# NVlabs/gbrl

Hardware: AMD Instinct MI355X
Metric: trees-fit/sec + predict rows/sec at batch=2^20, feat=128, depth=6, out=8 (higher is better)
Workload: dtype int32 fixed-point sums / f32 scores

## Files before the change

gbrl_amd/csrc/engine.h:

```cpp
#pragma once

#include <hip/hip_runtime.h>

#include <cstdint>
#include <stdexcept>
#include <array>
#include <initializer_list>
#include <chrono>
#include <cstring>
#include <string>
#include <unordered_map>
#include <vector>

#include "kernels.h"
#include "model.h"

namespace gbrl {

struct HipError : std::runtime_error { using std::runtime_error::runtime_error; };
struct NoDeviceError : std::runtime_error { using std::runtime_error::runtime_error; };
struct InvalidArgument : std::runtime_error { using std::runtime_error::runtime_error; };
struct Unsupported : std::runtime_error { using std::runtime_error::runtime_error; };

void hip_check(hipError_t e, const char *what);
// ... 233 lines not shown
    kern::PredictModel mirror_view();
    void finish(const char *launch, const char *phase, std::initializer_list<ReadBack> results);
    void run_predict(const PredictBatch &b, int start_tree, int stop_tree, float *out, bool out_dev);
    void run_continue(const PredictBatch &b, int start_tree, int stop_tree, const float *base, bool base_dev, float *out, bool out_dev);
    uint64_t cat_dict_token();
    void grow_tree(const detail::GrowCtx &c, std::vector<detail::HNode> &nodes, std::vector<int> &frontier, std::vector<int64_t> &acc,
                   double &leaf_scale);
    enum class SmallGrowth { Grown, NearTie, Unavailable };
    detail::StepTables upload_step_tables(const detail::GrowCtx &c, const detail::GrowDims &dims);
    SmallGrowth grow_small(const detail::GrowCtx &c, const detail::GrowDims &dims, const detail::StepTables &t, int blocks, detail::TreeBuilder &tb,
                           std::vector<int64_t> &acc, double &leaf_scale, const char *&why);
    void grow_levels(const detail::GrowCtx &c, const detail::GrowDims &dims, const detail::StepTables &t, detail::TreeBuilder &tb,
                     std::vector<int64_t> &acc, double &leaf_scale);
    detail::LevelWork level_workspace(const detail::GrowCtx &c, const detail::GrowDims &dims);
    void grow_levels_planned(const detail::GrowCtx &c, const detail::GrowDims &dims, const detail::StepTables &t, detail::LevelWork &w, detail::TreeBuilder &tb);
    void grow_levels_host(const detail::GrowCtx &c, const detail::GrowDims &dims, const detail::StepTables &t, detail::LevelWork &w, detail::TreeBuilder &tb,
                          detail::Stager &sta, detail::Stager &stb);
    detail::Level stage_level(const detail::GrowCtx &c, const detail::GrowDims &dims, detail::LevelWork &w, detail::TreeBuilder &tb, detail::Stager &sta, int depth,
                              std::vector<int> active);
    void level_histograms(const detail::GrowCtx &c, const detail::GrowDims &dims, const detail::LevelWork &w, const detail::Level &L);
    uint32_t score_select_level(const detail::GrowCtx &c, const detail::GrowDims &dims, const detail::StepTables &t, const detail::LevelWork &w, const detail::Level &L);
    void replay_near_ties(const detail::GrowCtx &c, const detail::GrowDims &dims, const detail::StepTables &t, const detail::LevelWork &w,
                          const std::vector<detail::HNode> &nodes, const detail::Level &L);
    void finish_leaves(const detail::GrowCtx &c, const detail::GrowDims &dims, const detail::LevelWork &w, detail::TreeBuilder &tb, detail::Stager &sta,
                       std::vector<int64_t> &acc, double &leaf_scale);
    uint32_t next_seq() { const uint32_t seq = ++level_seq_; return seq ? seq : ++level_seq_; }
    bool device_categorical_candidates(const char *dcells, const char *hcells, int N, int Fc, int B,
                                       std::vector<detail::CatCandidate> &cat_cands, std::vector<int> &cat_classes, bool launch_only = false,
                                       const float *dgrads = nullptr, int D = 0);
    void sharded_categorical_ranking(const char *hcat, const float *hgrads, int N, int Fc, int D, int B, std::vector<detail::CatCandidate> &cat_cands,
                                     std::vector<uint16_t> &h_catcodes, std::vector<int> &cat_classes);
    void numeric_thresholds(const float *dobs, int N, int F, int B, long long n_global, const uint32_t *d_kt, float *d_thr,
                            uint32_t *d_thrkeys, DevBuf &root_le_buf, const uint32_t **root_le_out, int pass1_chunks = 0, uint16_t *d_codes_out = nullptr,
                            bool *codes_written = nullptr);
    void read_step_hooks();
    bool fused_prep_applies(int N, int F, long long n_global) const;
    void check_prepared_model(const char *what) const;
    void check_prepared_dataset(const char *what, const PreparedDataset *ds) const;
    void step_prepared_run(const PreparedDataset *ds, const float *dgrads, const int32_t *d_rows, int m, const int32_t *cols = nullptr, int n_cols = 0);
    void begin_step_profile();
    void sync_code_bins(const PreparedDataset &ds);
    void check_code_range(const PreparedDataset &ds, const char *what, int start_tree, int stop_tree);
    kern::CodeTables sync_code_tables(const PreparedDataset &ds);
    NumericPrep prepare_numeric(PrepBuffers &pb, const float *dobs, int N, int F, int Fc, long long n_global, bool prep_candidate, detail::FusedStats *fs);
    void run_grad_stats(detail::FusedStats &g, int N, long long &n_global);
    void grow_step_tree(const detail::StepData &d, std::vector<detail::HNode> &nodes, std::vector<int> &frontier, std::vector<int64_t> &acc, double &leaf_scale);
// ... 207 lines not shown
```

gbrl_amd/csrc/engine_candidates.hip:

```cpp
#include "engine_step_detail.h"

namespace gbrl {

namespace detail {

void spin_until_published(volatile uint32_t *flag, uint32_t seq, hipStream_t s, const char *what) {
    const double kSpinSeconds = [] { const char *e = hooks::raw(hooks::SPIN_SECONDS); const double v = e ? std::atof(e) : 0.0; return v > 0.0 ? v : 120.0; }();
    int idle = 0;
    std::chrono::steady_clock::time_point t0;
    bool timed = false;
    for (unsigned spins = 1; *flag != seq; ++spins) {
        if ((spins & 0x3fff) == 0) {
            const hipError_t q = hipStreamQuery(s);
            if (q == hipSuccess) { if (++idle > 64) throw HipError(std::string("internal: ") + what + " were not published"); }
            else if (q != hipErrorNotReady) hip_check(q, what);
            if (!timed) { t0 = std::chrono::steady_clock::now(); timed = true; }
            else if (std::chrono::duration<double>(std::chrono::steady_clock::now() - t0).count() > kSpinSeconds) {
                hip_check(hipStreamSynchronize(s), what);
                if (*flag == seq) break;
                throw HipError(std::string("timeout: ") + what + " did not arrive (stream drained, nothing published)");
            }
        }
    }
    std::atomic_thread_fence(std::memory_order_acquire);
// ... 584 lines not shown
                bisection_quantiles(cum);
            } else if (!has_coll_ && !force_sample_select_ && !force_radix_ && kern::sort_quantiles_fits(N, B)) {
                int64_t *d_cum = upload_cum(cum);
                const bool no_fuse = [] { const char *e = hooks::raw(hooks::SORT_NO_CODES); return e && e[0] == '1'; }();
                uint16_t *cdst = no_fuse ? nullptr : d_codes_out;
                kern::sort_quantiles(d_kt, N, F, d_cum, B, d_thrkeys, d_thr, s, cdst);
                if (cdst && codes_written) *codes_written = true;
                floats_done = true;
                last_quantile_fallback_ = false;
            } else if (!force_sample_select_ && B <= kern::radix_max_targets() && n_global < (1ll << 32)) {
                int64_t *d_cum = upload_cum(cum);
                void *d_rs = d_radix_state_.ensure(kern::radix_state_bytes(F, B));
                uint32_t *d_rp = static_cast<uint32_t *>(d_radix_partial_.ensure(kern::radix_partial_bytes(F)));
                uint32_t *d_rl = static_cast<uint32_t *>(d_qlists_.ensure(kern::radix_list_bytes(N, F)));
                kern::RadixComm comm{};
                if (has_coll_) {
                    comm.ctx = this;
                    comm.allreduce_sum_i64 = &Engine::radix_exchange_trampoline;
                    comm.stream_ordered = rccl_comm_ != nullptr;
                    comm.gbuf = static_cast<int64_t *>(d_counts_.ensure(sizeof(int64_t) * kern::radix_exchange_words(F)));
                    comm.partial_global = static_cast<uint32_t *>(d_radix_global_.ensure(kern::radix_global_partial_bytes(F)));
                }
                uint32_t *d_le = has_coll_ ? nullptr : static_cast<uint32_t *>(root_le_buf.ensure(sizeof(uint32_t) * (static_cast<size_t>(F) * B + F)));
                const int rc = kern::radix_select(d_kt, N, F, d_cum, B, d_rs, d_rp, d_rl, d_thrkeys, s, has_coll_ ? &comm : nullptr, pass1_chunks, d_le);
                if (root_le_out) *root_le_out = d_le;
                if (rc != 0) throw HipError(rc == 2 ? "allreduce failed" : "radix select failed");
                last_quantile_fallback_ = false;
            } else {
                fast_quantile = true;
                kern::QuantilePlan plan = kern::quantile_plan(N);
                if (has_coll_) { plan.sample = 4096; plan.n_split = kern::kQuantileMaxSplit; }
                const size_t all_keys = static_cast<size_t>(N) * F;
                const uint32_t max_elems = static_cast<uint32_t>(B > 256 ? all_keys : std::min<size_t>(all_keys, std::max<size_t>(1u << 20, all_keys / 4)));
                int64_t *d_cum = upload_cum(cum);
                uint32_t *d_split = static_cast<uint32_t *>(d_splitters_.ensure(sizeof(uint32_t) * 2 * static_cast<size_t>(F) * kern::kQuantileMaxSplit));
                uint32_t *d_split_bfs = d_split + static_cast<size_t>(F) * kern::kQuantileMaxSplit;
                uint32_t *d_cc = static_cast<uint32_t *>(d_ccounts_.ensure(sizeof(uint32_t) * static_cast<size_t>(plan.n_chunks) * F * kern::kQuantileClasses));
                uint32_t *d_coff = static_cast<uint32_t *>(d_c2l_.ensure(sizeof(uint32_t) * F * kern::kQuantileClasses));
                uint32_t *d_toff = static_cast<uint32_t *>(d_tgt_list_.ensure(sizeof(uint32_t) * 2 * static_cast<size_t>(F) * B));
                uint32_t *d_tlen = d_toff + static_cast<size_t>(F) * B;
                uint32_t *d_tr = static_cast<uint32_t *>(d_tgt_rank_.ensure(sizeof(uint32_t) * F * B));
                uint32_t *d_lists = static_cast<uint32_t *>(d_qlists_.ensure(sizeof(uint32_t) * max_elems));
                hip_check(hipMemsetAsync(d_coff, 0xff, sizeof(uint32_t) * F * kern::kQuantileClasses, s), "memset");
                hip_check(hipMemsetAsync(d_qflags, 0, sizeof(uint32_t) * 4, s), "memset");
                int64_t *d_gcounts = nullptr;
                if (has_coll_) {
                    const int S = 4096, SU = S * coll_.world_size;
// ... 65 lines not shown
```

gbrl_amd/csrc/engine_grow_detail.h:

```cpp
#pragma once
#include "engine_step_detail.h"

namespace gbrl {
namespace detail {

struct GrowDims {
    GrowDims(const GrowCtx &c, bool has_coll, int world_size, int rank, Engine::Parity parity);
    int max_front, max_nodes, max_chunks;
    bool l2_degenerate;
    size_t table_cap, stage_bytes;
    int hist_chunk_budget, hist_max_chunks;
    size_t n_acc, hist_node_elems, feat_elems;
    int coll_P, coll_Fs, coll_lo, own_slots;
    size_t ar_max_bytes;
    int am_parts;
    size_t am_cap;
    size_t res_bytes;
    bool near_on;
    float near_rel;
    int near_max_rows;
    bool reference_asked;
    bool event_results;
};

// ... 55 lines not shown
    std::vector<HCond> in_cond_;
};

struct LevelWork {
    int32_t *rows[2];
    int32_t *rows_scratch;
    bool iota_root = false;
    int cur = 0;
    bool ar_prefix = false;
    int32_t *partials;
    int64_t *hist_lvl[2];
    int64_t *hist_coll, *hist_recv, *gather;
    float *scores, *parent, *am_v, *am_s;
    int32_t *am_i, *am_n;
    int32_t *cursors;
    int64_t *leafacc;
    ResultBlock d_res;
    ResultBlock h_res;
    volatile uint32_t *h_flag;
    void *h_res_dev;
    uint32_t *d_flag;
    unsigned *d_pub_done;
    NodeSplit *resolved;
};

struct Level {
    int depth = 0, n_act = 0;
    std::vector<int> active, compute_ids;
    std::vector<int32_t> slot_map;
    ChunkTable hist;
    std::vector<Chunk> count_chunks, part_chunks;
    bool hist_direct = false, root_countless = false, ar_level = false, drop_derived = false;
    int root_mode = 1, lvl_slots = 0, lvl_lo = 0;
    int64_t *d_hist = nullptr;
    const int64_t *d_hist_prev = nullptr;
    Chunk *d_chunks, *d_count_chunks, *d_part_chunks;
    int32_t *d_chunk_begin, *d_slotmap, *d_sub_par, *d_sub_sib, *d_path_len, *d_path_slot, *d_path_bin, *d_isroot, *d_seg_starts, *d_n_locals;
    float *d_path_val;
};

}
}
```

gbrl_amd/csrc/engine_grow_levels.hip:

```cpp
#include "engine_grow_detail.h"

namespace gbrl {

using namespace detail;

void Engine::grow_levels(const GrowCtx &c, const GrowDims &dims, const StepTables &t, TreeBuilder &tb, std::vector<int64_t> &acc, double &leaf_scale) {
    hipStream_t s = stream_;
    const bool device_plan = c.oblivious && !has_coll_ && device_levels_requested() && c.MD > 0 && c.MD <= 11  &&
                             c.n_cand > 0 && !dims.l2_degenerate;
    Stager sta(pin_a_, d_stage_a_, dims.stage_bytes, s), stb(pin_b_, d_stage_b_, dims.stage_bytes, s);
    LevelWork w = level_workspace(c, dims);
    tb.reset(dims.max_nodes);
    kern::publish_pair(c.d_thr, c.pub_thr_dev, c.pub_thr_bytes, c.d_scales, c.pub_scales_dev, sizeof(kern::StepScales), s);
    if (device_plan) grow_levels_planned(c, dims, t, w, tb);
    else if (c.n_cand > 0 && !dims.l2_degenerate) grow_levels_host(c, dims, t, w, tb, sta, stb);
    finish_leaves(c, dims, w, tb, sta, acc, leaf_scale);
}

LevelWork Engine::level_workspace(const GrowCtx &c, const GrowDims &dims) {
    hipStream_t s = stream_;
    const int N = c.N, D = c.D, max_front = dims.max_front;
    LevelWork w{};
    w.rows[0] = static_cast<int32_t *>(d_rows_[0].ensure(sizeof(int32_t) * N));
    w.rows[1] = static_cast<int32_t *>(d_rows_[1].ensure(sizeof(int32_t) * N));
// ... 110 lines not shown
    hip_check(hipMemcpyAsync(h_res_all, d_res_all, res_bytes * MD, hipMemcpyDeviceToHost, s), "D2H tree results");
    hip_check(hipStreamSynchronize(s), "sync tree");
    hip_check(hipGetLastError(), "growth kernels");
    for (int depth = 0; depth < MD; ++depth) {
        const std::vector<int> active = tb.frontier;
        if (static_cast<int>(active.size()) != (1 << depth)) throw HipError("internal: level size mismatch");
        LevelOutcome lvl = tb.digest_level(active, level_block(h_res_all, depth), DigestMode{});
        if (lvl.stop || lvl.splitting.empty()) { if (!lvl.stop) tb.frontier.clear(); break; }
        w.cur ^= 1;
        tb.frontier = lvl.next;
    }
}

void Engine::grow_levels_host(const GrowCtx &c, const GrowDims &dims, const StepTables &t, LevelWork &w, TreeBuilder &tb, Stager &sta, Stager &stb) {
    hipStream_t s = stream_;
    const int N = c.N;
    for (int depth = 0; depth < c.MD; ++depth) {
        std::vector<int> active = tb.active_nodes();
        if (active.empty()) break;
        const Level L = stage_level(c, dims, w, tb, sta, depth, std::move(active));
        level_histograms(c, dims, w, L);
        const uint32_t seq = score_select_level(c, dims, t, w, L);
        if (dims.event_results) hip_check(hipEventRecord(ev_level_, s), "hipEventRecord");
        phase_begin();
        if (!L.part_chunks.empty())
            kern::partition_rows(w.rows[w.cur], w.rows[w.cur ^ 1], c.d_codes, c.d_kt, N, L.d_part_chunks, static_cast<int>(L.part_chunks.size()), w.resolved, w.cursors, s);
        phase_end("partition");
        if (dims.event_results) {
            for (;;) {
                const hipError_t q = hipEventQuery(ev_level_);
                if (q == hipSuccess) break;
                if (q != hipErrorNotReady) hip_check(q, "hipEventQuery(level results)");
            }
        } else {
            verify_pending_categories();
            spin_until_published(w.h_flag, seq, s, "level results");
        }
        hip_check(hipGetLastError(), "growth kernels");
        if (w.am_s != nullptr && !has_coll_ && !dims.event_results) replay_near_ties(c, dims, t, w, tb.nodes, L);
        LevelOutcome lvl = tb.digest_level(L.active, w.h_res, DigestMode{});
        if (lvl.stop) break;
        stb.reset();
        if (!lvl.new_leaves.empty()) {
            const ChunkTable leaves = make_chunks(tb.nodes, lvl.new_leaves, 1024, true);
            if (!leaves.chunks.empty()) {
                Chunk *d_lc = stb.put(leaves.chunks.data(), leaves.chunks.size());
                stb.flush();
                phase_begin();
                kern::leaf_sums(c.dgrads, c.D, w.rows[w.cur], d_lc, static_cast<int>(leaves.chunks.size()), c.d_scales, w.leafacc, s);
                phase_end("leaves");
            }
        }
        if (lvl.splitting.empty()) { tb.frontier.clear(); break; }
        w.cur ^= 1;
        if (w.iota_root) { w.rows[0] = w.rows_scratch; w.iota_root = false; }
        tb.frontier = lvl.next;
    }
}

Level Engine::stage_level(const GrowCtx &c, const GrowDims &dims, LevelWork &w, TreeBuilder &tb, Stager &sta, int depth, std::vector<int> active) {
    std::vector<HNode> &nodes = tb.nodes;
    Level L;
    L.depth = depth;
    L.active = std::move(active);
    const std::vector<int> &act = L.active;
    const int n_act = L.n_act = static_cast<int>(act.size());
// ... 228 lines not shown
        io.pos = static_cast<int32_t *>(d_near_pos_.ensure(sizeof(int32_t) * rows17));
        io.nr = static_cast<int32_t *>(d_near_nrb_.ensure(sizeof(int32_t) * blocks17));
        io.vals = static_cast<float *>(d_near_vals_.ensure(sizeof(float) * rows17 * D));
        io.means = static_cast<float *>(d_near_means_.ensure(sizeof(float) * blocks17 * 2 * D));
        io.sums = static_cast<float *>(d_near_sums_.ensure(sizeof(float) * blocks17 * 2 * D));
        io.rowsort = static_cast<int32_t *>(d_near_rowsort_.ensure(sizeof(int32_t) * static_cast<size_t>(N)));
        io.tiles = static_cast<int32_t *>(d_near_tiles_.ensure(sizeof(int32_t) * kern::near_tie_fast_tiles(N, n_act)));
        io.seq_blocks = kern::near_tie_fast_blocks(N, D, n_act);
        io.chains_bytes = kern::near_tie_fast_chain_bytes(N, D, n_act);
        io.chains = d_near_chains_.ensure(io.chains_bytes);
    }
    kern::near_tie_replay(io, s);
    const uint32_t seq = next_seq();
    kern::resolve_splits(w.am_v, w.am_i, oblivious ? dims.am_parts : own_slots, w.d_res.best_idx(), w.d_res.best_score(), oblivious, n_act, t.ref_to_internal, t.cand_slot, t.slots, L.d_hist, nullptr, Fp, NB, D, w.resolved,
                         w.d_res.counts(), max_front, L.d_seg_starts, w.cursors, c.d_thrkeys, B, s, w.h_res_dev, w.d_flag, seq, w.d_pub_done,
                         L.drop_derived ? L.d_hist_prev : nullptr, L.drop_derived ? L.d_sub_par : nullptr, L.drop_derived ? L.d_sub_sib : nullptr, nullptr);
    if (!L.part_chunks.empty())
        kern::partition_rows(w.rows[w.cur], w.rows[w.cur ^ 1], c.d_codes, c.d_kt, N, L.d_part_chunks, static_cast<int>(L.part_chunks.size()), w.resolved, w.cursors, s);
    phase_end("near_tie_replay");
    spin_until_published(w.h_flag, seq, s, "level results after the near-tie replay");
    hip_check(hipGetLastError(), "near-tie replay kernels");
}

void Engine::finish_leaves(const GrowCtx &c, const GrowDims &dims, const LevelWork &w, TreeBuilder &tb, Stager &sta, std::vector<int64_t> &acc, double &leaf_scale) {
    hipStream_t s = stream_;
    const int D = c.D;
    std::vector<HNode> &nodes = tb.nodes;
    std::vector<int> last;
    for (int id : tb.frontier)
        if (!nodes[id].leaf) { nodes[id].leaf = true; last.push_back(id); }
    if (nodes.size() == 1) nodes[0].leaf = true;
    const ChunkTable leaves = make_chunks(nodes, last, 1024, true);
    if (!leaves.chunks.empty()) {
        sta.reset();
        Chunk *d_lc = sta.put(leaves.chunks.data(), leaves.chunks.size());
        sta.flush();
        phase_begin();
        kern::leaf_sums(c.dgrads, D, w.rows[w.cur], d_lc, static_cast<int>(leaves.chunks.size()), c.d_scales, w.leafacc, s);
        phase_end("leaves");
    }
    const size_t n_acc_words = nodes.size() * (D + 1);
    if (has_coll_) exchange(Red::SumI64, w.leafacc, n_acc_words);
    const size_t acc_bytes = sizeof(int64_t) * std::max<size_t>(1, n_acc_words);
    char *h_acc_raw = static_cast<char *>(pin_acc_.ensure(acc_bytes + 64));
    int64_t *h_acc = reinterpret_cast<int64_t *>(h_acc_raw);
    if (dims.event_results) {
        hip_check(hipMemcpyAsync(h_acc, w.leafacc, sizeof(int64_t) * n_acc_words, hipMemcpyDeviceToHost, s), "D2H leaf acc");
        hip_check(hipStreamSynchronize(s), "sync");
    } else {
        void *h_acc_dev = nullptr;
        hip_check(hipHostGetDevicePointer(&h_acc_dev, h_acc_raw, 0), "hipHostGetDevicePointer");
        volatile uint32_t *h_aflag = reinterpret_cast<volatile uint32_t *>(h_acc_raw + acc_bytes);
        const uint32_t seq = next_seq();
        *h_aflag = 0;
// ... 12 lines not shown
```

gbrl_amd/csrc/hooks.h:

```cpp
#pragma once
#include <cstdlib>

namespace gbrl {
namespace hooks {

#define GBRL_HIP_HOOKS(X) \
    X(BIN_PLAIN) \
    X(CAT_CHECK) \
    X(CAT_PROF) \
    X(CONTINUE_GENERIC) \
    X(DEVICE_LEVELS) \
    X(EVENT_RESULTS) \
    X(FORCE_BISECTION) \
    X(FORCE_COLLECTIVE) \
    X(HIST_ALLREDUCE_MAX_KB) \
    X(HIST_GENERIC) \
    X(HIST_PIPE) \
    X(HOST_CATEGORICAL) \
    X(KEEP_LAST_DERIVED) \
    X(LEAVES_GENERIC) \
    X(NEARTIE_DEBUG) \
    X(NEARTIE_MAX_ROWS) \
    X(NEARTIE_REL) \
    X(NEARTIE_SERIAL) \
    X(NO_DIRECT_HIST) \
    X(NO_IOTA_CACHE) \
    X(NO_NEARTIE_REPLAY) \
    X(NO_SMALL_GROW) \
    X(NO_SMALL_PREP) \
    X(NO_SMALL_STATS) \
    X(PREDICT_CHAIN) \
    X(PREDICT_GENERIC) \
    X(PREDICT_GRD_STREAM_MIN_ROWS) \
    X(PREDICT_GRD_STREAM_WAVES) \
    X(PREDICT_NB) \
    X(PREDICT_NOSPLIT) \
    X(PREDICT_NO_GRD_STREAM) \
    X(PREDICT_NO_PC) \
    X(PREDICT_NO_PERSIST) \
    X(PREDICT_NO_REG) \
    X(PREDICT_NO_RESIDENT) \
    X(PREDICT_OBL1) \
    X(PREDICT_REG_GROUPED) \
    X(PREDICT_REG_MIN_ROWS) \
    X(PREDICT_REG_ONLY) \
    X(PREDICT_REG_WAVES) \
    X(PREDICT_RG) \
    X(PREDICT_SCHED_MIN_ROWS) \
    X(PREDICT_TT) \
    X(QUANTILE_RADIX) \
    X(QUANTILE_SAMPLE) \
    X(RADIX_PLAIN_LOADS) \
    X(REFIT_GENERIC) \
    X(ROOT_COUNTS) \
    X(SHAP_DEVICE_ONLY) \
    X(SHAP_HOST) \
    X(SMALL_GROW_BLOCKS) \
    X(SMALL_GROW_PROF) \
    X(SMALL_PREP_PROF) \
    X(SORT_NO_CODES) \
    X(SPIN_SECONDS) \
    X(STAGED_GENERIC) \
    X(TEST_CAT_CLASH) \
    X(TEST_SMALL_GROW_FAIL) \
    X(TRANSPOSE_COUNT) \
    X(TRANSPOSE_PLAIN)

enum Id : int {
#define X(n) n,
    GBRL_HIP_HOOKS(X)
#undef X
    kCount
};

void begin_call();
const char *raw(Id id);
const char *name(Id id);
inline bool on(Id id) { const char *e = raw(id); return e && e[0] == '1'; }
inline int num(Id id, int dflt) { const char *e = raw(id); return e ? std::atoi(e) : dflt; }

}
}
```

gbrl_amd/csrc/kernels.h:

```cpp
#pragma once

#include <hip/hip_runtime.h>

#include <cstddef>
#include <cstdint>
#include <vector>

namespace gbrl {
namespace kern {

struct PerDeviceOnce {
    uint64_t done = 0;
    bool first() {
        int d = 0;
        if (hipGetDevice(&d) != hipSuccess || d < 0 || d >= 64) return true;
        if ((done >> d) & 1ull) return false;
        done |= 1ull << d;
        return true;
    }
};


struct Chunk {
    int32_t slot;
// ... 95 lines not shown
void select_update(uint32_t *prefix, const int64_t *counts, const uint32_t *tgt_off, const uint32_t *tgt_rank, int bit, int n_targets,
                   uint32_t *thr_keys, hipStream_t s);
void quantile_extract(const uint32_t *kt, int n, int F, const QuantilePlan &p, const uint32_t *splitters_bfs, const uint32_t *class_off,
                      const uint32_t *partial, uint32_t *out, hipStream_t s);
void quantile_select(const uint32_t *lists, const uint32_t *tgt_off, const uint32_t *tgt_len, const uint32_t *tgt_rank, int n_targets,
                     uint32_t *thr_keys, hipStream_t s);
int sort_quantiles_max_rows();
bool sort_quantiles_fits(int n, int B);
void sort_quantiles(const uint32_t *kt, int n, int F, const int64_t *cum, int B, uint32_t *thr_keys, float *thr_floats , hipStream_t s, uint16_t *codes = nullptr );
size_t radix_state_bytes(int F, int B);
size_t radix_partial_bytes(int F);
int radix_max_targets();
size_t radix_list_bytes(int n, int F);
struct RadixComm {
    void *ctx;
    int (*allreduce_sum_i64)(void *ctx, int64_t *dev_buf, size_t count);
    bool stream_ordered;
    int64_t *gbuf;
    uint32_t *partial_global;
};
size_t radix_exchange_words(int F);
size_t radix_global_partial_bytes(int F);
int radix_select(const uint32_t *kt, int n, int F, const int64_t *cum, int B, void *state, uint32_t *partial, uint32_t *lists,
                 uint32_t *thr_keys, hipStream_t s, const RadixComm *comm ,
                 int pass1_chunks = 0 ,
                 uint32_t *le_out = nullptr );
int transpose_keys_count(const float *obs, int n, int F, uint32_t *kt, uint32_t *partial, hipStream_t s);
void bin_cols(const uint32_t *kt, int n, int F, const uint32_t *thr_keys, int B, uint16_t *codes, hipStream_t s);
void scatter_cat_codes_grouped(const uint16_t *cat_codes, int n, int Fc, int F, uint16_t *codes, hipStream_t s);
constexpr int kCodeGroup = 16;
void gather_code_records(const uint16_t *codes , int n, int n_groups , const int32_t *rows , int m,
                         uint16_t *out , hipStream_t s);
void bin_like(const float *obs, int n, int F, const uint32_t *thr_keys, int B, uint16_t *codes , hipStream_t s);
void rows_minmax(const int32_t *rows, int m, int32_t *mm , hipStream_t s);
constexpr int kGatherColsRows = 64, kGatherColsMaxStaged = 16;
struct GatherColsPlan {
    int n_cols, n_out_groups, n_chunks, max_staged;
    int chunks_at, groups_at, offs_at, cols_at;
    size_t n_words, staged_groups;
};
GatherColsPlan gather_cols_plan(const int32_t *cols, int n_cols, std::vector<int32_t> &words);
void gather_code_columns(const uint16_t *codes , int n, const int32_t *rows , int m, const int32_t *d_plan,
                         const GatherColsPlan &p, uint16_t *out , hipStream_t s);
void gather_threshold_rows(const float *thr, const uint32_t *thr_keys, int B, const int32_t *d_plan, const GatherColsPlan &p, float *thr_out, uint32_t *keys_out,
                           hipStream_t s);
constexpr int kSampleRowsPerBlock = 2048, kSampleScanWidth = 512;
int sample_rows_blocks(int n);
// ... 173 lines not shown
    unsigned *sync;
    char *res;
    char *res_dev;
    int64_t *acc;
    uint32_t *status;
    uint32_t seq;
    uint32_t *prof = nullptr;
    StepScales *scales_out = nullptr;
    void *near_scratch = nullptr;
    const float *meanden = nullptr;
    bool resume = false;
    bool replay = false;
    float near_rel = 0.0f;
};
bool small_grow_supported(int N, int D, int NB, int MD, int n_slots, int n_cand);
int small_grow_blocks(int n_slots);
size_t small_grow_bests_bytes(int MD, int G, bool oblivious);
size_t small_grow_res_stride(int MD);
size_t small_grow_near_bytes(int G, int N, int MD);
bool small_grow(const SmallGrowIO &io, hipStream_t s);

void leaf_sums(const float *grads, int D, const int32_t *rows, const Chunk *chunks, int n_chunks, const StepScales *sc,
               int64_t *acc , hipStream_t s);

struct PredictModel {
    const int32_t *tree_indices, *depths, *feature_indices, *cat_ids;
    const float *feature_values, *values, *bias;
    const uint8_t *is_numerics, *inequality_directions;
    int n_trees, n_leaves, max_depth, D, oblivious;
    int n_opts;
    const int32_t *opt_start, *opt_stop;
    const float *opt_lr;
    const int32_t *cond_pack;
    const int32_t *grd_nodes;
    const int32_t *grd_node_off;
    int grd_ok, grd_max_nodes, grd_max_leaves;
    int obl_ok, coef_ok;
    uint64_t coef_cover;
    float coef[64];
    const float *rate;
    uint8_t owner[64];
    float *partial;
    size_t partial_floats;
    int tree_chunk;
    int tree_splits;
    int par_th;
// ... 131 lines not shown
```

gbrl_amd/csrc/kernels.hip:

```cpp
#include "kernels.h"
#include "hooks.h"
#include "kernels_common.h"
#include "score_common.h"
#include "small_prep.h"

#include <hip/hip_ext.h>

#include <algorithm>
#include <cmath>
#include <stdexcept>
#include <cstdlib>

namespace gbrl {
namespace kern {

namespace {

template <bool FACTOR>
__global__ void k_column_sums(const float *__restrict__ g, size_t n_el, int D, const float *__restrict__ center,
                              double *__restrict__ partials , const float *__restrict__ factor,
                              const int32_t *__restrict__ labels) {
    extern __shared__ double sh[];
    const int bs = blockDim.x;
    const int col = threadIdx.x % D;
// ... 1254 lines not shown
            int r[8];
            float g[8];
#pragma unroll
            for (int u = 0; u < 8; ++u) r[u] = rows[ck.start + p + u * per];
#pragma unroll
            for (int u = 0; u < 8; ++u) g[u] = grads[static_cast<size_t>(r[u]) * D + d];
#pragma unroll
            for (int u = 0; u < 8; ++u) s += __double2ll_rn(static_cast<double>(g[u]) * scale);
        }
        for (; p < ck.len; p += per) {
            const int row = rows[ck.start + p];
            s += __double2ll_rn(static_cast<double>(grads[static_cast<size_t>(row) * D + d]) * scale);
        }
        atomicAdd(&shl[d], static_cast<unsigned long long>(s));
    }
    __syncthreads();
    for (int i = threadIdx.x; i < D; i += blockDim.x)
        atomicAdd(reinterpret_cast<unsigned long long *>(&acc[static_cast<size_t>(ck.slot) * (D + 1) + i]), shl[i]);
    if (threadIdx.x == 0)
        atomicAdd(reinterpret_cast<unsigned long long *>(&acc[static_cast<size_t>(ck.slot) * (D + 1) + D]),
                  static_cast<unsigned long long>(ck.len));
}

}


int column_sums_blocks(int n, int D) { return grid_for(static_cast<size_t>(n) * D, 256 * 8, 1024); }

void column_sums(const float *g, int n, int D, const float *center, double *block_partials, int n_blocks, double *out,
                 hipStream_t s) {
    const int bs = D <= 256 ? (256 / D) * D : D;
    hipLaunchKernelGGL(k_column_sums<false>, dim3(n_blocks), dim3(bs), 2 * bs * sizeof(double), s, g, static_cast<size_t>(n) * D, D,
                       center, block_partials, static_cast<const float *>(nullptr), static_cast<const int32_t *>(nullptr));
    hipLaunchKernelGGL(k_column_sums_final, dim3(2 * D), dim3(256), 0, s, block_partials, n_blocks, D, out);
}

void column_sums_weighted(const float *g, const int32_t *labels, const float *factor, int n, int D, double *block_partials, int n_blocks, double *out,
                          hipStream_t s) {
    const int bs = D <= 256 ? (256 / D) * D : D;
    hipLaunchKernelGGL(k_column_sums<true>, dim3(n_blocks), dim3(bs), 2 * bs * sizeof(double), s, g, static_cast<size_t>(n) * D, D,
                       static_cast<const float *>(nullptr), block_partials, factor, labels);
    hipLaunchKernelGGL(k_column_sums_final, dim3(2 * D), dim3(256), 0, s, block_partials, n_blocks, D, out);
}

bool small_stats(const float *g, int n, int D, bool centred, int chunk_rows, double *stat, float *meanden, StepScales *sc, int32_t *qg, hipStream_t s) {
    const int n_blocks = column_sums_blocks(n, D);
// ... 539 lines not shown
        pl.path_slot[k * kMaxPath + q] = s_cslot[q];
        pl.path_val[k * kMaxPath + q] = s_cval[q];
        pl.path_bin[k * kMaxPath + q] = s_cbin[q];
    }
}
void plan_oblivious_level(int level, int n_rows, int chunk_rows, int budget, const NodeSplit *resolved_prev, const float *best_score_prev,
                          const float *thr, int B, const ObliviousPlan &pl, hipStream_t s) {
    hipLaunchKernelGGL(k_plan_oblivious, dim3(1), dim3(kPlanThreads), 0, s, level, n_rows, chunk_rows, budget, resolved_prev, best_score_prev, thr, B, pl);
}

void partition_rows(const int32_t *rows_in, int32_t *rows_out, const uint16_t *codes, const uint32_t *kt, int n_rows, const Chunk *chunks,
                    int n_chunks, const NodeSplit *splits, int32_t *cursors, hipStream_t s) {
    hipLaunchKernelGGL(k_partition, dim3(n_chunks), dim3(kPartThreads), 0, s, rows_in, rows_out, codes, kt, n_rows, chunks, splits,
                       cursors);
}

void leaf_sums(const float *grads, int D, const int32_t *rows, const Chunk *chunks, int n_chunks, const StepScales *sc, int64_t *acc,
               hipStream_t s) {
    const int bs = D <= 256 ? 256 : ((D + 63) / 64) * 64;
    hipLaunchKernelGGL(k_leaf_sums, dim3(n_chunks), dim3(bs), (D + 1) * sizeof(unsigned long long), s, grads, D, rows, chunks,
                       sc, acc);
}

}
}
```

gbrl_amd/csrc/radix_select.hip:

```cpp
#include "kernels.h"
#include "hooks.h"

#include <algorithm>
#include <cstdlib>
#include <vector>

namespace gbrl {
namespace kern {

namespace {

constexpr int kBins1 = 4096;
constexpr int kNone = 0xffff;
constexpr int kRadixThreads = 1024;
constexpr int kMaxTargets = 256;
constexpr int kChunks1 = 8;
constexpr int kCopies1 = 4;
constexpr int kChunksN = 8;
constexpr int kFiltWords = 1024, kFiltShift = 17;
constexpr int kSlotStride = 128;

__host__ __device__ constexpr int radix_bins(int pass) { return pass == 1 ? kBins1 : (pass == 4 ? 64 : 128); }
__host__ __device__ constexpr int radix_shift(int pass) { return pass == 1 ? 20 : (pass == 2 ? 13 : (pass == 3 ? 6 : 0)); }

// ... 235 lines not shown

constexpr int kTgtThreads = 1024;

__device__ __forceinline__ uint32_t wave_scan_incl(uint32_t v) {
    const int lane = threadIdx.x & 63;
#pragma unroll
    for (int d = 1; d < 64; d <<= 1) { const uint32_t t = __shfl_up(v, d); if (lane >= d) v += t; }
    return v;
}
__device__ __forceinline__ uint32_t block_scan_incl(uint32_t v, uint32_t *scratch ) {
    const int lane = threadIdx.x & 63, w = threadIdx.x >> 6;
    v = wave_scan_incl(v);
    if (lane == 63) scratch[w] = v;
    __syncthreads();
    uint32_t base = 0;
    for (int i = 0; i < w; ++i) base += scratch[i];
    __syncthreads();
    return v + base;
}

__global__ __launch_bounds__(kTgtThreads) void k_radix_targets(int pass, const uint32_t *__restrict__ partial, int n_chunks,
                                                               const int64_t *__restrict__ cum, int B, RadixState st,
                                                               uint32_t *__restrict__ thr_keys, int p1_u16, uint32_t *__restrict__ le_out,
                                                               const int64_t *__restrict__ gbuf , int F) {
    extern __shared__ uint32_t sums[];
    __shared__ int tslot[kMaxTargets], tdig[kMaxTargets];
    __shared__ uint32_t scratch[16], total_slots;
    const int f = blockIdx.x, k = threadIdx.x, lane = threadIdx.x & 63, wave = threadIdx.x >> 6;
    const int NB = radix_bins(pass);
    const int n_slots = pass == 1 ? 1 : static_cast<int>(st.n_slots[f * 4 + (pass - 2)]);
    const size_t pstride = pass == 1 ? kBins1 : kMaxTargets * kSlotStride;
    const uint32_t *p0 = partial + static_cast<size_t>(f) * n_chunks * pstride;
    if (pass == 1) {
        uint4 v = make_uint4(0, 0, 0, 0);
        if (gbuf) {
            v = *reinterpret_cast<const uint4 *>(gbuf + static_cast<size_t>(f) * (kBins1 / 2) + 2 * k);
        } else if (p1_u16) {
            const uint16_t *q0 = reinterpret_cast<const uint16_t *>(partial) + static_cast<size_t>(f) * n_chunks * kBins1 + k * 4;
            int c = 0;
            for (; c + 8 <= n_chunks; c += 8) {
                uint2 t[8];
#pragma unroll
                for (int u = 0; u < 8; ++u) t[u] = *reinterpret_cast<const uint2 *>(q0 + static_cast<size_t>(c + u) * kBins1);
#pragma unroll
                for (int u = 0; u < 8; ++u) { v.x += t[u].x & 0xffffu; v.y += t[u].x >> 16; v.z += t[u].y & 0xffffu; v.w += t[u].y >> 16; }
            }
            for (; c < n_chunks; ++c) {
// ... 27 lines not shown
    }
    __syncthreads();
    int slot = 0, digit = 0;
    uint32_t rank = 0, prefix = 0;
    if (k < B) {
        if (pass == 1) {
            rank = static_cast<uint32_t>(cum[k]);
        } else {
            slot = st.tgt_slot[static_cast<size_t>(f) * B + k];
            rank = st.tgt_rank[static_cast<size_t>(f) * B + k];
            prefix = st.tgt_prefix[static_cast<size_t>(f) * B + k];
        }
        const uint32_t *hs = sums + slot * NB;
        int lo = 0, hi = NB - 1;
        while (lo < hi) { const int mid = (lo + hi) >> 1; if (hs[mid] < rank) lo = mid + 1; else hi = mid; }
        digit = lo;
        if (pass == 1 && k == 0 && le_out) le_out[static_cast<size_t>(gridDim.x) * B + f] = sums[7];
        const uint32_t le_here = static_cast<uint32_t>(static_cast<uint64_t>(cum[k]) - rank + hs[lo]);
        rank -= lo ? hs[lo - 1] : 0u;
        prefix |= static_cast<uint32_t>(digit) << radix_shift(pass);
        if (pass == 4 && le_out) le_out[static_cast<size_t>(f) * B + k] = prefix < 0x007fffffu ? le_out[static_cast<size_t>(gridDim.x) * B + f] : le_here;
    }
    if (pass == 4) {
        if (k < B) thr_keys[static_cast<size_t>(f) * B + k] = prefix;
        return;
    }
    if (k < kMaxTargets) { tslot[k] = k < B ? slot : -1; tdig[k] = digit; }
    __syncthreads();
    const bool opens = (k < B) && (k == 0 || tslot[k - 1] != slot || tdig[k - 1] != digit);
    const bool new_parent = (k < B) && (k == 0 || tslot[k - 1] != slot);
    const uint32_t incl = block_scan_incl(opens ? 1u : 0u, scratch);
    const int my_slot = static_cast<int>(incl) - 1;
    if (k == B - 1) total_slots = incl;
    if (k < B) {
        st.tgt_slot[static_cast<size_t>(f) * B + k] = static_cast<uint16_t>(my_slot);
        st.tgt_rank[static_cast<size_t>(f) * B + k] = rank;
        st.tgt_prefix[static_cast<size_t>(f) * B + k] = prefix;
    }
    if (pass == 1) {
        uint16_t *m = st.map1 + static_cast<size_t>(f) * kBins1;
        for (int i = threadIdx.x; i < kBins1; i += kTgtThreads) m[i] = kNone;
        __syncthreads();
        if (opens) m[digit] = static_cast<uint16_t>(my_slot);
    } else {
        uint16_t *off = st.child_off + (static_cast<size_t>(f) * 2 + (pass - 2)) * 258;
        unsigned long long *bits = reinterpret_cast<unsigned long long *>(st.child_bits) + (static_cast<size_t>(f) * 2 + (pass - 2)) * 512;
        for (int i = threadIdx.x; i < 2 * n_slots; i += kTgtThreads) bits[i] = 0ull;
// ... 27 lines not shown
            }
        gbuf[i] = static_cast<int64_t>(static_cast<uint64_t>(a) | (static_cast<uint64_t>(b) << 32));
    }
}
constexpr size_t align16(size_t v) { return (v + 15) & ~static_cast<size_t>(15); }

}

size_t radix_state_bytes(int F, int B) {
    const size_t f = static_cast<size_t>(F);
    return align16(f * kBins1 * 2) + align16(f * 2 * 258 * 2) + align16(f * 2 * 512 * 8) + align16(f * 4 * 4) + align16(f * B * 2) +
           2 * align16(f * B * 4) + align16(f * kChunksN * 4);
}
size_t radix_list_bytes(int n, int F) { return sizeof(uint32_t) * (static_cast<size_t>(F) * (static_cast<size_t>(n) / 4 + 64) + 64); }
size_t radix_partial_bytes(int F) {
    const size_t a = static_cast<size_t>(F) * kChunks1 * kBins1, b = static_cast<size_t>(F) * kChunksN * kMaxTargets * kSlotStride;
    return sizeof(uint32_t) * (a > b ? a : b);
}
int radix_max_targets() { return kMaxTargets; }
size_t radix_exchange_words(int F) { return static_cast<size_t>(kMaxTargets) * F * (kSlotStride / 2); }
size_t radix_global_partial_bytes(int F) { return sizeof(uint32_t) * static_cast<size_t>(F) * kMaxTargets * kSlotStride; }

int radix_select(const uint32_t *kt, int n, int F, const int64_t *cum, int B, void *state, uint32_t *partial, uint32_t *lists,
                 uint32_t *thr_keys, hipStream_t s, const RadixComm *comm, int pass1_chunks, uint32_t *le_out) {
    char *p = static_cast<char *>(state);
    auto take = [&](size_t bytes) { char *q = p; p += align16(bytes); return q; };
    const size_t f = static_cast<size_t>(F);
    RadixState st;
    st.map1 = reinterpret_cast<uint16_t *>(take(f * kBins1 * 2));
    st.child_off = reinterpret_cast<uint16_t *>(take(f * 2 * 258 * 2));
    st.child_bits = reinterpret_cast<uint64_t *>(take(f * 2 * 512 * 8));
    st.n_slots = reinterpret_cast<uint32_t *>(take(f * 4 * 4));
    st.tgt_slot = reinterpret_cast<uint16_t *>(take(f * B * 2));
    st.tgt_rank = reinterpret_cast<uint32_t *>(take(f * B * 4));
    st.tgt_prefix = reinterpret_cast<uint32_t *>(take(f * B * 4));
    st.list_cnt = reinterpret_cast<uint32_t *>(take(f * kChunksN * 4));
    st.lists = lists;
    const size_t aux = kBins1 * 2 + 2 * 512 * 8 + 2 * 260 * 2 + kFiltWords * 4 + (kRadixThreads / 64) * 128 * 4;
    const size_t lds1 = static_cast<size_t>(kCopies1) * kBins1 * 4 + aux, lds23 = static_cast<size_t>(kMaxTargets) * 128 * 4 + aux,
                 lds4 = static_cast<size_t>(kMaxTargets) * 64 * 4 + aux;
    static PerDeviceOnce attr;
    if (attr.first()) {
        (void)hipFuncSetAttribute(reinterpret_cast<const void *>(k_radix_count<2>), hipFuncAttributeMaxDynamicSharedMemorySize, static_cast<int>(lds23));
        (void)hipFuncSetAttribute(reinterpret_cast<const void *>(k_radix_count<3>), hipFuncAttributeMaxDynamicSharedMemorySize, static_cast<int>(lds23));
        (void)hipFuncSetAttribute(reinterpret_cast<const void *>(k_radix_count<4>), hipFuncAttributeMaxDynamicSharedMemorySize, static_cast<int>(lds4));
        (void)hipFuncSetAttribute(reinterpret_cast<const void *>(k_radix_targets), hipFuncAttributeMaxDynamicSharedMemorySize, kMaxTargets * 128 * 4);
    }
// ... 9 lines not shown
        if (comm) {
            int rows = 1;
            hipLaunchKernelGGL(k_radix_globalize, dim3(1024), dim3(256), 0, s, pass, partial, n_chunks_pass, F, st, comm->gbuf, p1_u16);
            p1_u16 = 0;
            if (comm->stream_ordered) {
                if (pass >= 2) rows = std::min(B, kMaxTargets);
            } else {
                if (pass >= 2) {
                    h_slots.resize(static_cast<size_t>(F) * 4);
                    if (hipMemcpyAsync(h_slots.data(), st.n_slots, sizeof(uint32_t) * h_slots.size(), hipMemcpyDeviceToHost, s) != hipSuccess) return 1;
                }
                if (hipStreamSynchronize(s) != hipSuccess) return 1;
                if (pass >= 2) {
                    rows = 0;
                    for (int f2 = 0; f2 < F; ++f2) rows = std::max(rows, static_cast<int>(h_slots[f2 * 4 + (pass - 2)]));
                }
            }
            const size_t words = static_cast<size_t>(rows) * F * (radix_bins(pass) / 2);
            if (comm->allreduce_sum_i64(comm->ctx, comm->gbuf, words) != 0) return 2;
            chunks = 1;
        }
        const size_t lds = pass == 1 ? kBins1 * 4 : static_cast<size_t>(kMaxTargets) * radix_bins(pass) * 4;
        hipLaunchKernelGGL(k_radix_targets, dim3(F), dim3(kTgtThreads), lds, s, pass, src, chunks, cum, B, st, thr_keys, p1_u16, le_out,
                           comm ? comm->gbuf : nullptr, F);
        return 0;
    };
    int rc = 0;
    const bool plain_loads = [] { const char *e = hooks::raw(hooks::RADIX_PLAIN_LOADS); return e && e[0] == '1'; }();
    if (pass1_chunks > 0) {
        if ((rc = finish_pass(1, pass1_chunks)) != 0) return rc;
    } else {
        hipLaunchKernelGGL(k_radix_count<1>, dim3(c1, F), dim3(kRadixThreads), lds1, s, kt, n, c1, B, st, partial, plain_loads);
        if ((rc = finish_pass(1, c1)) != 0) return rc;
    }
    hipLaunchKernelGGL(k_radix_count<2>, dim3(cn, F), dim3(kRadixThreads), lds23, s, kt, n, cn, B, st, partial, plain_loads);
    if ((rc = finish_pass(2, cn)) != 0) return rc;
    hipLaunchKernelGGL(k_radix_count<3>, dim3(cn, F), dim3(kRadixThreads), lds23, s, kt, n, cn, B, st, partial, plain_loads);
    if ((rc = finish_pass(3, cn)) != 0) return rc;
    hipLaunchKernelGGL(k_radix_count<4>, dim3(cn, F), dim3(kRadixThreads), lds4, s, kt, n, cn, B, st, partial, plain_loads);
    return finish_pass(4, cn);
}

int transpose_keys_count(const float *obs, int n, int F, uint32_t *kt, uint32_t *partial, hipStream_t s) {
    const char *env_off = hooks::raw(hooks::TRANSPOSE_COUNT);
    const bool off = env_off && env_off[0] == '0';
    const int chunks = (n + kTcChunk - 1) / kTcChunk;
    if (off || n < (1 << 16) || (n & 3) || (F & 3) || chunks > kTcMaxChunks || (reinterpret_cast<uintptr_t>(obs) & 15) ||
// ... 22 lines not shown
```

Measured before the change: 541.6.

## Fuse last-level partition with leaf sums and emit float thresholds from radix select

At the final depth, the row partition kernel and the separate leaf-sum pass are replaced by one kernel. It evaluates each node's split per row and accumulates left/right gradient sums and counts directly into the leaf accumulators. Those results are published to pinned host memory, so the host spins on a flag instead of launching another pass, and the host checks row counts against the expected node sizes. The radix-select targets kernel now also writes float thresholds, which removes a separate key-to-float conversion step, and it clamps small keys. This adds a new code path with more complex bookkeeping and relies on 64-bit atomics in shared memory.

```diff
diff --git a/gbrl_amd/csrc/engine.h b/gbrl_amd/csrc/engine.h
--- a/gbrl_amd/csrc/engine.h
+++ b/gbrl_amd/csrc/engine.h
@@ -279,6 +279,7 @@
     uint32_t score_select_level(const detail::GrowCtx &c, const detail::GrowDims &dims, const detail::StepTables &t, const detail::LevelWork &w, const detail::Level &L);
     void replay_near_ties(const detail::GrowCtx &c, const detail::GrowDims &dims, const detail::StepTables &t, const detail::LevelWork &w,
                           const std::vector<detail::HNode> &nodes, const detail::Level &L);
+    void enqueue_last_level(const detail::GrowCtx &c, detail::LevelWork &w, const detail::TreeBuilder &tb, const detail::Level &L);
     void finish_leaves(const detail::GrowCtx &c, const detail::GrowDims &dims, const detail::LevelWork &w, detail::TreeBuilder &tb, detail::Stager &sta,
                        std::vector<int64_t> &acc, double &leaf_scale);
     uint32_t next_seq() { const uint32_t seq = ++level_seq_; return seq ? seq : ++level_seq_; }
diff --git a/gbrl_amd/csrc/engine_candidates.hip b/gbrl_amd/csrc/engine_candidates.hip
--- a/gbrl_amd/csrc/engine_candidates.hip
+++ b/gbrl_amd/csrc/engine_candidates.hip
@@ -630,7 +630,8 @@
                     comm.partial_global = static_cast<uint32_t *>(d_radix_global_.ensure(kern::radix_global_partial_bytes(F)));
                 }
                 uint32_t *d_le = has_coll_ ? nullptr : static_cast<uint32_t *>(root_le_buf.ensure(sizeof(uint32_t) * (static_cast<size_t>(F) * B + F)));
-                const int rc = kern::radix_select(d_kt, N, F, d_cum, B, d_rs, d_rp, d_rl, d_thrkeys, s, has_coll_ ? &comm : nullptr, pass1_chunks, d_le);
+                const int rc = kern::radix_select(d_kt, N, F, d_cum, B, d_rs, d_rp, d_rl, d_thrkeys, d_thr, s, has_coll_ ? &comm : nullptr, pass1_chunks, d_le);
+                floats_done = true;
                 if (root_le_out) *root_le_out = d_le;
                 if (rc != 0) throw HipError(rc == 2 ? "allreduce failed" : "radix select failed");
                 last_quantile_fallback_ = false;
diff --git a/gbrl_amd/csrc/engine_grow_detail.h b/gbrl_amd/csrc/engine_grow_detail.h
--- a/gbrl_amd/csrc/engine_grow_detail.h
+++ b/gbrl_amd/csrc/engine_grow_detail.h
@@ -101,6 +101,15 @@
     uint32_t *d_flag;
     unsigned *d_pub_done;
     NodeSplit *resolved;
+    struct LastLevel {
+        bool on = false;
+        int base_nodes = 0, n_act = 0;
+        uint32_t seq = 0;
+        volatile uint32_t *h_flag = nullptr;
+        const int64_t *h_acc = nullptr;
+        std::vector<int> node;
+        std::vector<long long> rows;
+    } last;
 };
 
 struct Level {
diff --git a/gbrl_amd/csrc/engine_grow_levels.hip b/gbrl_amd/csrc/engine_grow_levels.hip
--- a/gbrl_amd/csrc/engine_grow_levels.hip
+++ b/gbrl_amd/csrc/engine_grow_levels.hip
@@ -156,10 +156,15 @@
         level_histograms(c, dims, w, L);
         const uint32_t seq = score_select_level(c, dims, t, w, L);
         if (dims.event_results) hip_check(hipEventRecord(ev_level_, s), "hipEventRecord");
+        const bool fuse_last = depth == c.MD - 1 && !has_coll_ && !dims.event_results && w.am_s == nullptr && !L.part_chunks.empty() &&
+                               kern::split_leaf_sums_supported(c.D) && tb.nodes.size() + 2 * static_cast<size_t>(L.n_act) <= static_cast<size_t>(dims.max_nodes) &&
+                               !hooks::on(hooks::NO_FUSED_LAST_LEVEL) ;
         phase_begin();
-        if (!L.part_chunks.empty())
+        if (fuse_last)
+            enqueue_last_level(c, w, tb, L);
+        else if (!L.part_chunks.empty())
             kern::partition_rows(w.rows[w.cur], w.rows[w.cur ^ 1], c.d_codes, c.d_kt, N, L.d_part_chunks, static_cast<int>(L.part_chunks.size()), w.resolved, w.cursors, s);
-        phase_end("partition");
+        phase_end(fuse_last ? "last_level_leaves" : "partition");
         if (dims.event_results) {
             for (;;) {
                 const hipError_t q = hipEventQuery(ev_level_);
@@ -173,9 +178,23 @@
         hip_check(hipGetLastError(), "growth kernels");
         if (w.am_s != nullptr && !has_coll_ && !dims.event_results) replay_near_ties(c, dims, t, w, tb.nodes, L);
         LevelOutcome lvl = tb.digest_level(L.active, w.h_res, DigestMode{});
+        if (fuse_last) {
+            w.last.node.assign(2 * static_cast<size_t>(L.n_act), -1);
+            w.last.rows.assign(2 * static_cast<size_t>(L.n_act), 0);
+            for (int k = 0; k < L.n_act; ++k) {
+                const HNode &nd = tb.nodes[L.active[k]];
+                if (nd.left >= 0) {
+                    w.last.node[2 * k] = nd.left; w.last.rows[2 * k] = tb.nodes[nd.left].n_local;
+                    w.last.node[2 * k + 1] = nd.right; w.last.rows[2 * k + 1] = tb.nodes[nd.right].n_local;
+                } else {
+                    w.last.node[2 * k] = nd.depth == 0 ? -1 : L.active[k];
+                    w.last.rows[2 * k] = nd.n_local;
+                }
+            }
+        }
         if (lvl.stop) break;
         stb.reset();
-        if (!lvl.new_leaves.empty()) {
+        if (!lvl.new_leaves.empty() && !fuse_last) {
             const ChunkTable leaves = make_chunks(tb.nodes, lvl.new_leaves, 1024, true);
             if (!leaves.chunks.empty()) {
                 Chunk *d_lc = stb.put(leaves.chunks.data(), leaves.chunks.size());
@@ -450,6 +469,26 @@
     hip_check(hipGetLastError(), "near-tie replay kernels");
 }
 
+void Engine::enqueue_last_level(const GrowCtx &c, LevelWork &w, const TreeBuilder &tb, const Level &L) {
+    hipStream_t s = stream_;
+    const int W = c.D + 1;
+    LevelWork::LastLevel &ll = w.last;
+    ll.on = true;
+    ll.base_nodes = static_cast<int>(tb.nodes.size());
+    ll.n_act = L.n_act;
+    kern::split_leaf_sums(c.dgrads, c.D, w.rows[w.cur], c.d_codes, c.d_kt, c.N, L.d_part_chunks, static_cast<int>(L.part_chunks.size()), w.resolved, c.d_scales,
+                          w.leafacc + static_cast<size_t>(ll.base_nodes) * W, s);
+    const size_t acc_bytes = sizeof(int64_t) * (static_cast<size_t>(ll.base_nodes) + 2 * static_cast<size_t>(ll.n_act)) * W;
+    char *h_acc_raw = static_cast<char *>(pin_acc_.ensure(acc_bytes + 64));
+    void *h_acc_dev = nullptr;
+    hip_check(hipHostGetDevicePointer(&h_acc_dev, h_acc_raw, 0), "hipHostGetDevicePointer");
+    ll.h_acc = reinterpret_cast<const int64_t *>(h_acc_raw);
+    ll.h_flag = reinterpret_cast<volatile uint32_t *>(h_acc_raw + acc_bytes);
+    ll.seq = next_seq();
+    *ll.h_flag = 0;
+    kern::publish_block(w.leafacc, h_acc_dev, acc_bytes, reinterpret_cast<uint32_t *>(static_cast<char *>(h_acc_dev) + acc_bytes), ll.seq, s, true);
+}
+
 void Engine::finish_leaves(const GrowCtx &c, const GrowDims &dims, const LevelWork &w, TreeBuilder &tb, Stager &sta, std::vector<int64_t> &acc, double &leaf_scale) {
     hipStream_t s = stream_;
     const int D = c.D;
@@ -458,6 +497,25 @@
     for (int id : tb.frontier)
         if (!nodes[id].leaf) { nodes[id].leaf = true; last.push_back(id); }
     if (nodes.size() == 1) nodes[0].leaf = true;
+    if (w.last.on) {
+        const LevelWork::LastLevel &ll = w.last;
+        const size_t W = static_cast<size_t>(D) + 1;
+        spin_until_published(ll.h_flag, ll.seq, s, "leaf sums");
+        leafacc_clean_ptr_ = w.leafacc;
+        acc.assign(nodes.size() * W, 0);
+        std::copy(ll.h_acc, ll.h_acc + static_cast<size_t>(ll.base_nodes) * W, acc.begin());
+        const long long off = hooks::on(hooks::TEST_LAST_LEVEL_COUNTS) ? 1 : 0;
+        for (size_t q = 0; q < ll.node.size(); ++q) {
+            const int64_t *src = ll.h_acc + (static_cast<size_t>(ll.base_nodes) + q) * W;
+            if (src[D] != ll.rows[q] + off)
+                throw HipError("internal: last level, node " + std::to_string(q / 2) + " side " + std::to_string(q % 2) + ": " + std::to_string(src[D]) +
+                               " rows summed, " + std::to_string(ll.rows[q] + off) + " expected");
+            if (ll.node[q] >= 0) std::copy(src, src + W, acc.begin() + static_cast<size_t>(ll.node[q]) * W);
+        }
+        if (!std::isfinite(c.h_scales->hmax_build) || !std::isfinite(c.h_scales->hmax_raw)) throw InvalidArgument("non-finite gradients");
+        leaf_scale = c.h_scales->leaf_scale;
+        return;
+    }
     const ChunkTable leaves = make_chunks(nodes, last, 1024, true);
     if (!leaves.chunks.empty()) {
         sta.reset();
diff --git a/gbrl_amd/csrc/hooks.h b/gbrl_amd/csrc/hooks.h
--- a/gbrl_amd/csrc/hooks.h
+++ b/gbrl_amd/csrc/hooks.h
@@ -24,6 +24,7 @@
     X(NEARTIE_REL) \
     X(NEARTIE_SERIAL) \
     X(NO_DIRECT_HIST) \
+    X(NO_FUSED_LAST_LEVEL) \
     X(NO_IOTA_CACHE) \
     X(NO_NEARTIE_REPLAY) \
     X(NO_SMALL_GROW) \
@@ -62,6 +63,7 @@
     X(SPIN_SECONDS) \
     X(STAGED_GENERIC) \
     X(TEST_CAT_CLASH) \
+    X(TEST_LAST_LEVEL_COUNTS) \
     X(TEST_SMALL_GROW_FAIL) \
     X(TRANSPOSE_COUNT) \
     X(TRANSPOSE_PLAIN)
diff --git a/gbrl_amd/csrc/kernels.h b/gbrl_amd/csrc/kernels.h
--- a/gbrl_amd/csrc/kernels.h
+++ b/gbrl_amd/csrc/kernels.h
@@ -141,7 +141,8 @@
 size_t radix_exchange_words(int F);
 size_t radix_global_partial_bytes(int F);
 int radix_select(const uint32_t *kt, int n, int F, const int64_t *cum, int B, void *state, uint32_t *partial, uint32_t *lists,
-                 uint32_t *thr_keys, hipStream_t s, const RadixComm *comm ,
+                 uint32_t *thr_keys, float *thr , hipStream_t s,
+                 const RadixComm *comm ,
                  int pass1_chunks = 0 ,
                  uint32_t *le_out = nullptr );
 int transpose_keys_count(const float *obs, int n, int F, uint32_t *kt, uint32_t *partial, hipStream_t s);
@@ -361,6 +362,9 @@
 
 void leaf_sums(const float *grads, int D, const int32_t *rows, const Chunk *chunks, int n_chunks, const StepScales *sc,
                int64_t *acc , hipStream_t s);
+bool split_leaf_sums_supported(int D);
+void split_leaf_sums(const float *grads, int D, const int32_t *rows, const uint16_t *codes, const uint32_t *kt , int n_rows, const Chunk *chunks,
+                     int n_chunks, const NodeSplit *splits, const StepScales *sc, int64_t *acc , hipStream_t s);
 
 struct PredictModel {
     const int32_t *tree_indices, *depths, *feature_indices, *cat_ids;
diff --git a/gbrl_amd/csrc/kernels.hip b/gbrl_amd/csrc/kernels.hip
--- a/gbrl_amd/csrc/kernels.hip
+++ b/gbrl_amd/csrc/kernels.hip
@@ -1300,6 +1300,64 @@
                   static_cast<unsigned long long>(ck.len));
 }
 
+template <bool kKeys>
+__device__ __forceinline__ void split_leaf_rows(const float *__restrict__ grads, int D, const int32_t *__restrict__ rows, const uint16_t *__restrict__ codes,
+                                                const uint32_t *__restrict__ kt, int n_rows, const Chunk ck, bool split, int fslot, bool is_cat, int bin,
+                                                uint32_t thr_key, double scale, int per, int sub, int d, long long (&s)[2], int (&n)[2]) {
+    const uint32_t *kcol = kKeys ? kt + static_cast<size_t>(fslot) * n_rows : nullptr;
+    const uint16_t *cbase = kKeys ? nullptr : codes + (static_cast<size_t>(fslot >> 4) * n_rows) * kCodeGroup + (fslot & (kCodeGroup - 1));
+    for (int p = sub; p < ck.len; p += 8 * per) {
+        int r[8];
+        uint32_t key[8];
+        float g[8];
+#pragma unroll
+        for (int u = 0; u < 8; ++u) r[u] = rows[ck.start + min(p + u * per, ck.len - 1)];
+#pragma unroll
+        for (int u = 0; u < 8; ++u) key[u] = kKeys ? kcol[r[u]] : static_cast<uint32_t>(cbase[static_cast<size_t>(r[u]) * kCodeGroup]);
+#pragma unroll
+        for (int u = 0; u < 8; ++u) g[u] = grads[static_cast<size_t>(r[u]) * D + d];
+#pragma unroll
+        for (int u = 0; u < 8; ++u) {
+            if (p + u * per >= ck.len) continue;
+            const bool right = split && (kKeys ? key[u] > thr_key : (is_cat ? static_cast<int>(key[u]) == bin : static_cast<int>(key[u]) > bin));
+            s[right ? 1 : 0] += __double2ll_rn(static_cast<double>(g[u]) * scale);
+            n[right ? 1 : 0] += 1;
+        }
+    }
+}
+constexpr int kSplitLeafThreads = 1024;
+__global__ __launch_bounds__(kSplitLeafThreads) void k_split_leaf_sums(const float *__restrict__ grads, int D, const int32_t *__restrict__ rows,
+                                                                       const uint16_t *__restrict__ codes, const uint32_t *__restrict__ kt, int n_rows,
+                                                                       const Chunk *__restrict__ chunks, const NodeSplit *__restrict__ splits,
+                                                                       const StepScales *__restrict__ scp, int64_t *__restrict__ acc) {
+    extern __shared__ unsigned long long shl[];
+    const int W = D + 1;
+    const double scale = scp->leaf_scale;
+    for (int i = threadIdx.x; i < 2 * W; i += blockDim.x) shl[i] = 0ull;
+    __syncthreads();
+    const Chunk ck = chunks[blockIdx.x];
+    if (ck.len <= 0) return;
+    const NodeSplit sp = splits[ck.slot];
+    const bool split = sp.do_split != 0;
+    const int fslot = split ? sp.fslot : 0;
+    const int per = blockDim.x / D > 0 ? blockDim.x / D : 1;
+    const int d = threadIdx.x % D, sub = threadIdx.x / D;
+    if (sub < per) {
+        long long s[2] = {0, 0};
+        int n[2] = {0, 0};
+        if (split && !sp.is_cat && kt) split_leaf_rows<true>(grads, D, rows, codes, kt, n_rows, ck, split, fslot, false, sp.bin, sp.thr_key, scale, per, sub, d, s, n);
+        else split_leaf_rows<false>(grads, D, rows, codes, kt, n_rows, ck, split, fslot, sp.is_cat != 0, sp.bin, 0u, scale, per, sub, d, s, n);
+#pragma unroll
+        for (int side = 0; side < 2; ++side) {
+            if (s[side]) atomicAdd(&shl[side * W + d], static_cast<unsigned long long>(s[side]));
+            if (d == 0 && n[side]) atomicAdd(&shl[side * W + D], static_cast<unsigned long long>(n[side]));
+        }
+    }
+    __syncthreads();
+    for (int i = threadIdx.x; i < 2 * W; i += blockDim.x)
+        if (shl[i]) atomicAdd(reinterpret_cast<unsigned long long *>(&acc[static_cast<size_t>(ck.slot) * 2 * W + i]), shl[i]);
+}
+
 }
 
 
@@ -1885,5 +1943,12 @@
                        sc, acc);
 }
 
-}
-}
+bool split_leaf_sums_supported(int D) { return D >= 1 && D <= kSplitLeafThreads; }
+void split_leaf_sums(const float *grads, int D, const int32_t *rows, const uint16_t *codes, const uint32_t *kt, int n_rows, const Chunk *chunks, int n_chunks,
+                     const NodeSplit *splits, const StepScales *sc, int64_t *acc, hipStream_t s) {
+    hipLaunchKernelGGL(k_split_leaf_sums, dim3(n_chunks), dim3(kSplitLeafThreads), 2 * (D + 1) * sizeof(unsigned long long), s, grads, D, rows, codes, kt, n_rows,
+                       chunks, splits, sc, acc);
+}
+
+}
+}
diff --git a/gbrl_amd/csrc/radix_select.hip b/gbrl_amd/csrc/radix_select.hip
--- a/gbrl_amd/csrc/radix_select.hip
+++ b/gbrl_amd/csrc/radix_select.hip
@@ -281,7 +281,8 @@
 __global__ __launch_bounds__(kTgtThreads) void k_radix_targets(int pass, const uint32_t *__restrict__ partial, int n_chunks,
                                                                const int64_t *__restrict__ cum, int B, RadixState st,
                                                                uint32_t *__restrict__ thr_keys, int p1_u16, uint32_t *__restrict__ le_out,
-                                                               const int64_t *__restrict__ gbuf , int F) {
+                                                               const int64_t *__restrict__ gbuf , int F,
+                                                               float *__restrict__ thr_floats ) {
     extern __shared__ uint32_t sums[];
     __shared__ int tslot[kMaxTargets], tdig[kMaxTargets];
     __shared__ uint32_t scratch[16], total_slots;
@@ -355,7 +356,11 @@
         if (pass == 4 && le_out) le_out[static_cast<size_t>(f) * B + k] = prefix < 0x007fffffu ? le_out[static_cast<size_t>(gridDim.x) * B + f] : le_here;
     }
     if (pass == 4) {
-        if (k < B) thr_keys[static_cast<size_t>(f) * B + k] = prefix;
+        if (k < B) {
+            const uint32_t key = prefix < 0x007fffffu ? 0x007fffffu : prefix;
+            thr_keys[static_cast<size_t>(f) * B + k] = key;
+            thr_floats[static_cast<size_t>(f) * B + k] = __uint_as_float((key & 0x80000000u) ? (key & 0x7fffffffu) : ~key);
+        }
         return;
     }
     if (k < kMaxTargets) { tslot[k] = k < B ? slot : -1; tdig[k] = digit; }
@@ -429,7 +434,7 @@
 size_t radix_global_partial_bytes(int F) { return sizeof(uint32_t) * static_cast<size_t>(F) * kMaxTargets * kSlotStride; }
 
 int radix_select(const uint32_t *kt, int n, int F, const int64_t *cum, int B, void *state, uint32_t *partial, uint32_t *lists,
-                 uint32_t *thr_keys, hipStream_t s, const RadixComm *comm, int pass1_chunks, uint32_t *le_out) {
+                 uint32_t *thr_keys, float *thr, hipStream_t s, const RadixComm *comm, int pass1_chunks, uint32_t *le_out) {
     char *p = static_cast<char *>(state);
     auto take = [&](size_t bytes) { char *q = p; p += align16(bytes); return q; };
     const size_t f = static_cast<size_t>(F);
@@ -485,7 +490,7 @@
         }
         const size_t lds = pass == 1 ? kBins1 * 4 : static_cast<size_t>(kMaxTargets) * radix_bins(pass) * 4;
         hipLaunchKernelGGL(k_radix_targets, dim3(F), dim3(kTgtThreads), lds, s, pass, src, chunks, cum, B, st, thr_keys, p1_u16, le_out,
-                           comm ? comm->gbuf : nullptr, F);
+                           comm ? comm->gbuf : nullptr, F, thr);
         return 0;
     };
     int rc = 0;
```

After: 547.4 (median of 4 runs). About the same (+1.1%).
